# ZJU-FAST-Lab/Implicit-SDF-Planner

Measured on AMD Instinct MI355X. Metric: SDF cost+grad point-evals/sec, higher is better.
Workload: dtype f64; 1 GPU; V3 ESDF-tile sweep: 1 trajectory x 40 pieces x 65 samples/piece, 256^3 fp32 ESDF @ 0.2 m, kernel_size 21, box robot (1.6,0.3,0.3) central-diff grad, occ_thresh = 0, cull off = BASELINE configs[1]; pieces=40, samples_per_piece=65, grid=256, kernel_size=21, collective=none

## Files before the change

implicit-sdf-planner_amd/csrc/dev_math.hpp:

```cpp
#pragma once
#include <hip/hip_runtime.h>

namespace isdf {

template <typename T> struct v3 { T x, y, z; };
using d3 = v3<double>;
using f3 = v3<float>;
struct d4 { double w, x, y, z; };
struct m3 { double a[9]; };

template <typename T> __device__ __forceinline__ v3<T> mkv(T x, T y, T z) { v3<T> r; r.x = x; r.y = y; r.z = z; return r; }
__device__ __forceinline__ d3 mk3(double x, double y, double z) { return mkv<double>(x, y, z); }
template <typename T> __device__ __forceinline__ v3<T> operator+(v3<T> a, v3<T> b) { return mkv<T>(a.x + b.x, a.y + b.y, a.z + b.z); }
template <typename T> __device__ __forceinline__ v3<T> operator-(v3<T> a, v3<T> b) { return mkv<T>(a.x - b.x, a.y - b.y, a.z - b.z); }
template <typename T> __device__ __forceinline__ v3<T> operator*(T s, v3<T> a) { return mkv<T>(s * a.x, s * a.y, s * a.z); }
template <typename T> __device__ __forceinline__ T dot3(v3<T> a, v3<T> b) { return a.x * b.x + a.y * b.y + a.z * b.z; }

#ifdef ISDF_LEAN_MATH
__device__ __forceinline__ double m_sqrt(double x) {
    const double y = __builtin_amdgcn_rsq(fmax(fabs(x), 2.2250738585072014e-308));
    double g = x * y, h = 0.5 * y;
    const double r = fma(-h, g, 0.5);
    g = fma(g, r, g);
    h = fma(h, r, h);
// ... 155 lines not shown
    t.dzt1 = j.y + P.dh_over_m * t.dw1;
    t.dzt2 = j.z + P.dh_over_m * t.dw2;
    t.dz0 = t.ng00 * t.dzt0 + t.ng01 * t.dzt1 + t.ng02 * t.dzt2;
    t.dz1 = t.ng01 * t.dzt0 + t.ng11 * t.dzt1 + t.ng12 * t.dzt2;
    t.dz2 = t.ng02 * t.dzt0 + t.ng12 * t.dzt1 + t.ng22 * t.dzt2;
    t.omg_den = s.z2 + 1.0;
    [[maybe_unused]] const double inv_omg = m_rcp(t.omg_den);
    t.omg_term = ISDF_QUOT(t.dz2, t.omg_den, inv_omg);
}
__device__ __forceinline__ d3 flat_omg(const FlatS &s, const FlatS2 &t) {
    [[maybe_unused]] const double inv_omg = m_rcp(t.omg_den);
    return mk3(-t.dz1 + s.z1 * t.omg_term, t.dz0 - s.z0 * t.omg_term, ISDF_QUOT(s.z1 * t.dz0 - s.z0 * t.dz1, t.omg_den, inv_omg));
}

__device__ __forceinline__ void flat_backward_from(const FlatP &P, d3 v, d3 a, const FlatS &s, const FlatS2 &t, d3 pos_grad, d3 vel_grad,
                                                   d4 quat_grad, d3 omg_grad, d3 &gP, d3 &gV, d3 &gA, d3 &gJ) {
    [[maybe_unused]] const double inv_tilt = m_rcp(s.tilt_den), inv_omg = m_rcp(t.omg_den), inv_ng = m_rcp(t.ng_den), inv_zn = m_rcp(s.zu_norm), inv_cp = m_rcp(s.cp_term);
    const double tilt0b = quat_grad.w, tilt1b = quat_grad.x, tilt2b = quat_grad.y;
    [[maybe_unused]] const double tilt_den_sqr = s.tilt_den * s.tilt_den;
    const double tilt_denb = ISDF_QUOT(s.z1 * tilt1b - s.z0 * tilt2b, tilt_den_sqr, inv_tilt * inv_tilt) + 0.5 * tilt0b;
    const double omg_termb = -s.z0 * omg_grad.y + s.z1 * omg_grad.x;
    double tb = ISDF_QUOT(omg_grad.z, t.omg_den, inv_omg);
    double z1b = t.dz0 * tb;
    const double dz0b = s.z1 * tb + omg_grad.y;
    double z0b = -(t.dz1 * tb);
    const double dz1b = -s.z0 * tb - omg_grad.x;
    const double omg_denb = -ISDF_QUOT((s.z1 * t.dz0 - s.z0 * t.dz1) * tb, t.omg_den, inv_omg) - ISDF_QUOT(ISDF_QUOT(t.dz2 * omg_termb, t.omg_den, inv_omg), t.omg_den, inv_omg);
    tb = -(t.omg_term * omg_grad.y);
    z0b += tb;
    tb = -(t.omg_term * omg_grad.x);
    z0b += ISDF_QUOT(tilt2b, s.tilt_den, inv_tilt);
    z1b += -tb - ISDF_QUOT(tilt1b, s.tilt_den, inv_tilt);
    const double dz2b = ISDF_QUOT(omg_termb, t.omg_den, inv_omg);
    const double z2b = omg_denb + ISDF_QUOT(tilt_denb, s.tilt_den, inv_tilt);

    const double ng02b = t.dzt0 * dz2b + t.dzt2 * dz0b;
    const double dzt0b = t.ng02 * dz2b + t.ng01 * dz1b + t.ng00 * dz0b;
    const double ng12b = t.dzt1 * dz2b + t.dzt2 * dz1b;
    const double dzt1b = t.ng12 * dz2b + t.ng11 * dz1b + t.ng01 * dz0b;
    const double ng22b = t.dzt2 * dz2b;
    const double dzt2b = t.ng22 * dz2b + t.ng12 * dz1b + t.ng02 * dz0b;
    const double ng01b = t.dzt0 * dz1b + t.dzt1 * dz0b;
    const double ng11b = t.dzt1 * dz1b;
    const double ng00b = t.dzt0 * dz0b;
    gJ = mk3(dzt0b, dzt1b, dzt2b);
    const double dw0b = P.dh_over_m * dzt0b, dw1b = P.dh_over_m * dzt1b, dw2b = P.dh_over_m * dzt2b;
    tb = ISDF_QUOT(P.cp * (v.z * dw2b + v.y * dw1b + v.x * dw0b), s.cp_term, inv_cp);
    gA = mk3(s.w_term * dw0b + v.x * tb, s.w_term * dw1b + v.y * tb, s.w_term * dw2b + v.z * tb);
    gV = mk3(t.dw_term * dw0b + a.x * tb, t.dw_term * dw1b + a.y * tb, t.dw_term * dw2b + a.z * tb);
    double cp_termb = -ISDF_QUOT(t.v_dot_a * tb, s.cp_term, inv_cp);
    tb = ISDF_QUOT(ng22b, t.ng_den, inv_ng);
    double zs0b = tb, zs1b = tb;
    double ng_denb = -ISDF_QUOT((s.s0 + s.s1) * tb, t.ng_den, inv_ng);
    const double zu12b = -ISDF_QUOT(ng12b, t.ng_den, inv_ng);
    tb = ISDF_QUOT(ng11b, t.ng_den, inv_ng);
    ng_denb += ISDF_QUOT(ISDF_QUOT(t.zu12 * ng12b, t.ng_den, inv_ng), t.ng_den, inv_ng) - ISDF_QUOT((s.s0 + s.s2) * tb, t.ng_den, inv_ng);
    zs0b += tb;
    double zs2b = tb;
    const double zu02b = -ISDF_QUOT(ng02b, t.ng_den, inv_ng);
    const double zu01b = -ISDF_QUOT(ng01b, t.ng_den, inv_ng);
    tb = ISDF_QUOT(ng00b, t.ng_den, inv_ng);
    ng_denb += ISDF_QUOT(ISDF_QUOT(t.zu02 * ng02b, t.ng_den, inv_ng), t.ng_den, inv_ng) + ISDF_QUOT(ISDF_QUOT(t.zu01 * ng01b, t.ng_den, inv_ng), t.ng_den, inv_ng) - ISDF_QUOT((s.s1 + s.s2) * tb, t.ng_den, inv_ng);
    const double zu_normb = s.zu_sqr_norm * ng_denb - (s.zu2 * z2b + s.zu1 * z1b + s.zu0 * z0b) / s.zu_sqr_norm;
    const double zu_sqr_normb = s.zu_norm * ng_denb + ISDF_QUOT(0.5 * zu_normb, s.zu_norm, inv_zn);
    tb += zu_sqr_normb;
    zs1b += tb;
    zs2b += tb;
    const double zu2b = ISDF_QUOT(z2b, s.zu_norm, inv_zn) + s.zu0 * zu02b + s.zu1 * zu12b + 2 * s.zu2 * zs2b;
    const double w2b = P.dh_over_m * zu2b;
    const double zu1b = ISDF_QUOT(z1b, s.zu_norm, inv_zn) + s.zu2 * zu12b + s.zu0 * zu01b + 2 * s.zu1 * zs1b;
    const double w1b = P.dh_over_m * zu1b;
    zs0b += zu_sqr_normb;
    const double zu0b = ISDF_QUOT(z0b, s.zu_norm, inv_zn) + s.zu2 * zu02b + s.zu1 * zu01b + 2 * s.zu0 * zs0b;
    const double w0b = P.dh_over_m * zu0b;
    const double w_termb = a.z * dw2b + a.y * dw1b + a.x * dw0b + v.z * w2b + v.y * w1b + v.x * w0b;
    gA.x += zu0b; gA.y += zu1b; gA.z += zu2b;
    cp_termb += P.cp * w_termb;
    const double vsb = ISDF_QUOT(0.5 * cp_termb, s.cp_term, inv_cp);
    gV.x += s.w_term * w0b + 2 * v.x * vsb + vel_grad.x;
    gV.y += s.w_term * w1b + 2 * v.y * vsb + vel_grad.y;
    gV.z += s.w_term * w2b + 2 * v.z * vsb + vel_grad.z;
    gP = pos_grad;
}
__device__ __forceinline__ void flat_backward(const FlatP &P, d3 v, d3 a, d3 jer, d3 pos_grad, d3 vel_grad,
                                              d4 quat_grad, d3 omg_grad, d3 &gP, d3 &gV, d3 &gA, d3 &gJ) {
    FlatS s; FlatS2 t;
    flat_core(P, v, a, s);
    flat_core2(P, v, a, jer, s, t);
    flat_backward_from(P, v, a, s, t, pos_grad, vel_grad, quat_grad, omg_grad, gP, gV, gA, gJ);
}

struct Basis { double b0[6], b1[6], b2[6], b3[6], b4[6]; };
__device__ __forceinline__ void poly_basis(double s1, Basis &B) {
    const double s2 = s1 * s1, s3 = s2 * s1, s4 = s2 * s2, s5 = s4 * s1;
    B.b0[0] = 1.0; B.b0[1] = s1; B.b0[2] = s2; B.b0[3] = s3; B.b0[4] = s4; B.b0[5] = s5;
    B.b1[0] = 0.0; B.b1[1] = 1.0; B.b1[2] = 2.0 * s1; B.b1[3] = 3.0 * s2; B.b1[4] = 4.0 * s3; B.b1[5] = 5.0 * s4;
    B.b2[0] = 0.0; B.b2[1] = 0.0; B.b2[2] = 2.0; B.b2[3] = 6.0 * s1; B.b2[4] = 12.0 * s2; B.b2[5] = 20.0 * s3;
    B.b3[0] = 0.0; B.b3[1] = 0.0; B.b3[2] = 0.0; B.b3[3] = 6.0; B.b3[4] = 24.0 * s1; B.b3[5] = 60.0 * s2;
    B.b4[0] = 0.0; B.b4[1] = 0.0; B.b4[2] = 0.0; B.b4[3] = 0.0; B.b4[4] = 24.0; B.b4[5] = 120.0 * s1;
}
template <int K0 = 0> __device__ __forceinline__ d3 ct_beta(const double *__restrict__ c, int ld, const double *b) {
    d3 r;
    double s = 0.0;
#pragma unroll
    for (int k = K0; k < 6; k++) s += c[k] * b[k];
    r.x = s; s = 0.0;
#pragma unroll
    for (int k = K0; k < 6; k++) s += c[ld + k] * b[k];
    r.y = s; s = 0.0;
#pragma unroll
    for (int k = K0; k < 6; k++) s += c[2 * ld + k] * b[k];
    r.z = s;
    return r;
}

struct TrajView { const double *T; const double *C; int N; };
__device__ __forceinline__ int traj_locate(const TrajView &tr, double &t) {
    int idx = 0;
    bool walking = true;
    double last = 0.0;
    for (int k = 0; k < tr.N; k++) {
        const double dur = tr.T[k];
        last = dur;
        walking = walking && (t > dur);
        if (walking) { t -= dur; idx = k + 1; }
        if (!__builtin_amdgcn_ballot_w64(walking)) break;
    }
    if (idx == tr.N) { idx--; t += last; }
    return idx;
}
__device__ __forceinline__ void traj_eval(const TrajView &tr, int piece, double t, d3 &pos, d3 &vel, d3 &acc, d3 &jer) {
    pos = mk3(0, 0, 0); vel = pos; acc = pos; jer = pos;
    double pos_tn = 1.0, vel_tn = 1.0, acc_tn = 1.0, jer_tn = 1.0;
    int vel_n = 1, acc_m = 1, acc_n = 2, jl = 1, jm = 2, jn = 3;
    const int ld = 6 * tr.N;
    const double *c = tr.C + 6 * piece;
#pragma unroll
    for (int power = 0; power <= 5; power++) {
        const d3 ck = mk3(c[power], c[ld + power], c[2 * ld + power]);
        pos = pos + pos_tn * ck;
        pos_tn *= t;
        if (power >= 1) { vel = vel + (vel_n * vel_tn) * ck; vel_tn *= t; vel_n++; }
        if (power >= 2) { acc = acc + (acc_m * acc_n * acc_tn) * ck; acc_tn *= t; acc_m++; acc_n++; }
        if (power >= 3) { jer = jer + (jl * jm * jn * jer_tn) * ck; jer_tn *= t; jl++; jm++; jn++; }
    }
}

__device__ __forceinline__ double wave_sum(double v) {
#pragma unroll
    for (int off = 32; off >= 1; off >>= 1) v += __shfl_xor(v, off, 64);
    return v;
}

__device__ __forceinline__ int wave_sum8_lane(int k) { return ((k & 1) << 3) | (((k >> 1) & 1) << 4) | ((k >> 2) << 5); }
template <int CTRL> __device__ __forceinline__ double dpp_mov_f64(double v) {
    const int lo = __builtin_amdgcn_mov_dpp(__double2loint(v), CTRL, 0xf, 0xf, false);
    const int hi = __builtin_amdgcn_mov_dpp(__double2hiint(v), CTRL, 0xf, 0xf, false);
    return __hiloint2double(hi, lo);
}
__device__ __forceinline__ double swap32_sum(double a, double b) {
    const auto lo = __builtin_amdgcn_permlane32_swap(__double2loint(a), __double2loint(b), false, false);
    const auto hi = __builtin_amdgcn_permlane32_swap(__double2hiint(a), __double2hiint(b), false, false);
    return __hiloint2double(hi[0], lo[0]) + __hiloint2double(hi[1], lo[1]);
}
__device__ __forceinline__ double swap16_sum(double a, double b) {
    const auto lo = __builtin_amdgcn_permlane16_swap(__double2loint(a), __double2loint(b), false, false);
// ... 55 lines not shown
```

implicit-sdf-planner_amd/csrc/isdf_host.hip:

```cpp
#include "isdf_ctx.hpp"
#include "minco_dev.hpp"
#include "lbfgs_host.hpp"
#include <array>
#include <atomic>
#include <map>
#include <dlfcn.h>
#include <chrono>
#include <cmath>
#include <cstdio>
#include <cstring>
#include <functional>
#include <cstdlib>
#include <string>
#include <vector>
#include <new>
#include "fwn_host.hpp"

using namespace isdf;

namespace {
thread_local std::string g_create_error;
}

int isdf_fail(isdf_ctx *c, int code, const char *msg) {
// ... 741 lines not shown
        P.point_partial = c->d_point_partial; P.point_piece = c->d_point_piece; P.point_stat = c->d_point_stat;
        P.point_nr = c->d_point_nr; P.task_buf = c->d_task_buf; P.task_map = c->d_task_map; P.words = c->d_v1_words; P.point_lmask = c->d_point_lmask;
        const bool scan_lpt = !c->env_no_lpt && !fixed_tstar;
        const bool sort_here = c->shape.kind == ISDF_SHAPE_MESH;
        P.scan_ticks = scan_lpt ? c->d_scan_ticks : nullptr; P.scan_order_out = scan_lpt ? c->d_scan_order : nullptr; P.scan_sort_here = (scan_lpt && sort_here) ? 1 : 0;
        const bool order_valid = sort_here || (c->scan_order_b == (long long)b && c->scan_order_e == (long long)e && c->scan_order_epoch == c->points_epoch);
        P.scan_order = (scan_lpt && order_valid) ? c->d_scan_order : nullptr;
        const long long order_b = sort_here ? -1 : b, order_e = sort_here ? -1 : e;
        if (scan_lpt) { c->scan_order_b = c->scan_order_e = -1; }
        P.direct_records = fixed_tstar ? 1 : 0;
        { int rc2 = ensure(c, &c->d_hist, &c->hist_cap, (size_t)N); if (rc2) return rc2; }
        P.hist = c->d_hist;
        P.stats = c->d_stats;
        P.dbg = nullptr;
        if (const char *e = getenv("ISDF_DEBUG_TIMING")) if (e[0] == '1') {
            const size_t need = (size_t)c->M * 7 + (size_t)(N + 1) * 8;
            if (c->dbg_cap < need) {
                if (c->d_dbg) (void)hipFree(c->d_dbg);
                c->d_dbg = nullptr; c->dbg_cap = 0;
                HIPCHK(c, hipMalloc(&c->d_dbg, need * sizeof(unsigned long long)));
                c->dbg_cap = need;
            }
            HIPCHK(c, hipMemsetAsync(c->d_dbg, 0, need * sizeof(unsigned long long), st));
            c->dbg_used = need;
            P.dbg = c->d_dbg;
        }
        if (fixed_tstar) {
            launch_swept_fixed(P, d_tstar, st);
            launch_swept_reduce(P, d_out, st);
            HIPCHK(c, hipGetLastError());
            return ISDF_OK;
        }
        launch_swept_prepare(P, st);
        ProfEvent *ev;
        int rc = prof_begin(c, st, &ev);
        if (rc) return rc;
        launch_swept_sweep(P, st, ev ? ev->a : nullptr, ev ? ev->b : nullptr);
        const bool ev2 = ev && c->prof_secondary;
        if (ev2) { HIPCHK(c, hipEventRecord(ev->c, st)); }
        launch_swept_reduce(P, d_out, st);
        if (ev2) { HIPCHK(c, hipEventRecord(ev->d, st)); }
        HIPCHK(c, hipGetLastError());
        if (scan_lpt) { c->scan_order_b = order_b; c->scan_order_e = order_e; c->scan_order_epoch = c->points_epoch; }
        return ISDF_OK;
    }

    if (cfg.enable_pos && c->shape.kind == ISDF_SHAPE_MESH && c->mesh_depth > isdf::MESH_Q_LEVELS)
        return fail(c, ISDF_ERR_UNSUPPORTED, "mesh hierarchy deeper than 12 levels: the tile sweep (V2 / V3) does not take it (the swept-volume sweep does)");
    if (cfg.enable_pos) {
        if (!c->have_geom) return fail(c, ISDF_ERR_STATE, "grid not set");
        if (cfg.variant == ISDF_V3_ESDF_TILE && !c->d_esdf) return fail(c, ISDF_ERR_STATE, "V3 needs an ESDF grid");
        if (cfg.variant == ISDF_V2_OCC_TILE && !c->d_occ) return fail(c, ISDF_ERR_STATE, "V2 needs an occupancy grid");
    }
    const long long total_pieces = (long long)n_traj * N;
    long long pb, pe;
    shard_range(total_pieces, c->rank, c->world, pb, pe);
    const size_t n_samples = (size_t)total_pieces * (cfg.integral_intervs + 1);
    { int rc0 = isdf_reserve_sweep_buffers(c, total_pieces); if (rc0) return rc0; }
    int rc = ISDF_OK;
    SweepParams P{};
    P.grid = c->grid;
    if (!c->have_geom) { P.grid.X = P.grid.Y = P.grid.Z = 1; P.grid.res = 1.0; }
    P.shape = c->shape;
    fill_flat(cfg, P.flat);
    P.variant = cfg.variant; P.K = cfg.integral_intervs; P.enable_dyn = cfg.enable_dyn; P.enable_pos = cfg.enable_pos;
    P.enable_cull = cfg.enable_cull;
    P.n_traj = n_traj; P.N = N; P.piece_begin = (int)pb; P.piece_end = (int)pe;
    P.bd_half = cfg.kernel_size * P.grid.res / 2;
    P.safety_hor = cfg.safety_hor; P.weight_p = cfg.weight_p; P.weight_v = cfg.weight_v; P.weight_omg = cfg.weight_omg;
    P.weight_theta = cfg.weight_theta;
    P.vel_sqr_max = cfg.vmax * cfg.vmax; P.omg_sqr_max = cfg.omgmax * cfg.omgmax; P.theta_max = cfg.thetamax;
    P.mu = cfg.smoothing_eps; P.inv_mu = 1.0 / cfg.smoothing_eps; P.inv_K = 1.0 / cfg.integral_intervs;
    P.occ_thresh = (float)cfg.occ_thresh;
    P.cull_threshold = 0.0;
    if (cfg.variant == ISDF_V3_ESDF_TILE && cfg.enable_cull && c->shape.bound_radius > 0)
        P.cull_threshold = c->shape.bound_radius + cfg.safety_hor + std::sqrt(3.0) * P.grid.res + (cfg.occ_thresh > 0 ? cfg.occ_thresh : 0.0);
    P.T = d_T; P.coeffs = d_coeffs; P.acc = c->d_acc; P.sample_info = c->d_sample_info; P.piece_cost = c->d_piece_cost;
    P.out = d_out; P.stats = c->d_stats;
    P.dbg = nullptr;
    P.sample_map = (c->d_sample_map && c->sample_map_n == 4 * (((size_t)(pe - pb) * (cfg.integral_intervs + 1) + 3) / 4)) ? c->d_sample_map : nullptr;
    P.dbg_flags = 0;
    if (const char *e = getenv("ISDF_DEBUG_FLAGS")) P.dbg_flags = atoi(e);
    if (const char *e = getenv("ISDF_DEBUG_TIMING")) if (e[0] == '1') {
        const size_t need = n_samples * 8 + (size_t)total_pieces * 4 + 4;
        if (c->dbg_cap < need) {
            if (c->d_dbg) (void)hipFree(c->d_dbg);
            c->d_dbg = nullptr; c->dbg_cap = 0;
            HIPCHK(c, hipMalloc(&c->d_dbg, need * sizeof(unsigned long long)));
            c->dbg_cap = need;
        }
        HIPCHK(c, hipMemsetAsync(c->d_dbg, 0, need * sizeof(unsigned long long), st));
        c->dbg_used = need;
        P.dbg = c->d_dbg;
    }
    if (cfg.enable_pos && c->bits_dirty) {
        const int zw = (c->grid.Z + 31) / 32, xw = (c->grid.X + 31) / 32, yw = (c->grid.Y + 31) / 32;
        const size_t nwz = (size_t)c->grid.X * c->grid.Y * zw, nwx = (size_t)c->grid.Y * c->grid.Z * xw, nwy = (size_t)c->grid.X * c->grid.Z * yw;
        const size_t nw = nwz + nwx + nwy;
        if (c->bits_cap < nw) {
            if (c->d_bits) (void)hipFree(c->d_bits);
            c->d_bits = nullptr; c->bits_cap = 0;
            HIPCHK(c, hipMalloc(&c->d_bits, nw * sizeof(unsigned)));
            c->bits_cap = nw;
        }
        c->grid.ZW = zw; c->grid.XW = xw; c->grid.YW = yw;
        c->grid.bits = c->d_bits; c->grid.bits_x = c->d_bits + nwz; c->grid.bits_y = c->d_bits + nwz + nwx;
        launch_build_bits(c->grid, cfg.variant == ISDF_V3_ESDF_TILE ? 1 : 0, cfg.occ_thresh, c->d_bits, st);
        launch_build_bits_xy(c->grid, cfg.variant == ISDF_V3_ESDF_TILE ? 1 : 0, cfg.occ_thresh, c->d_bits + nwz, c->d_bits + nwz + nwx, st);
        c->bits_dirty = false;
        P.grid = c->grid;
    }
    c->last_P = P; c->have_last_P = true;
    ProfEvent *ev;
    rc = prof_begin(c, st, &ev);
    if (rc) return rc;
    if (ev && !cfg.enable_pos) { ev = nullptr; c->prof_used--; }
    const bool ev2 = ev && c->prof_secondary;
    const bool fused = c->fuse_small && !ev2 && sweep_can_fuse(P);
    {
        int xerr = ISDF_OK;
        if (isdf_xchg_fill(c, &P.xf, (size_t)total_pieces, &xerr)) {
            if (xerr != ISDF_OK) return xerr;
        }
    }
    if (hd) {
        if (!fused || P.xf.world > 1 || P.dbg) return ISDF_DIRECT_NA;
        { int rc1 = ensure_stage(c, (size_t)total_pieces); if (rc1) return rc1; }
        P.out = hd->out; P.host_flag = hd->flags; P.seq = hd->seq;
        if (!hd->via_bar) { P.host_T = hd->T; P.host_coeffs = hd->coeffs; P.stage = c->d_stage; P.stage_flags = c->d_stage_flags; }
        c->last_P = P;
    }
    P.plan_cls_in = nullptr; P.plan_cls_out = nullptr; P.plan_map_out = nullptr; P.plan_zone = 0; P.plan_group = 1;
    P.plan_lr_in = P.plan_hist_in = nullptr; P.plan_lr_out = P.plan_hist_out = nullptr;
    {
        const int K1 = cfg.integral_intervs + 1;
        const long long n_loc = pe - pb, ns_local = n_loc * K1;
        const int nb = (int)((ns_local + 3) / 4);
        P.n_sweep_blocks = nb;
        if (c->n_cus == 0) { hipDeviceProp_t pr; c->n_cus = (hipGetDeviceProperties(&pr, c->device) == hipSuccess && pr.multiProcessorCount > 0) ? pr.multiProcessorCount : 256; }
        const bool no_plan = c->env_no_lpt;
        bool plan = cfg.enable_pos && !no_plan && !P.sample_map && K1 <= 128 && nb > c->n_cus && ns_local < (1LL << 28) && c->shape.kind != ISDF_SHAPE_MESH;
        long long group = n_loc;
        int zone = 0;
        if (plan) {
            if (fused) {
                plan = P.xf.world <= 1 && pb == 0 && pe == total_pieces && ns_local <= PLAN_GROUP_MAX_SAMPLES;
                zone = c->n_cus;
            } else if (nb <= sweep_resident_blocks(P, c->n_cus) && ns_local <= PLAN_GROUP_MAX_SAMPLES) {
                zone = c->n_cus;
            } else if (ns_local > PLAN_GROUP_MAX_SAMPLES) {
                group = N;
                plan = (long long)N * K1 <= PLAN_GROUP_MAX_SAMPLES && pb % N == 0 && pe % N == 0;
            }
        }
        if (!plan) c->plan_k = 0;
        else {
            const size_t ns_cap = (size_t)4 * nb, np_cap = (size_t)n_loc;
            if (c->plan_ns_cap < ns_cap || c->plan_np_cap < np_cap) {
                HIPCHK(c, hipStreamSynchronize(st));
                for (void *q : {(void *)c->d_plan_cls, (void *)c->d_plan_map, (void *)c->d_plan_lr, (void *)c->d_plan_hist}) if (q) (void)hipFree(q);
                c->d_plan_cls = nullptr; c->d_plan_map = nullptr; c->d_plan_lr = nullptr; c->d_plan_hist = nullptr;
                c->plan_ns_cap = c->plan_np_cap = 0; c->plan_k = 0; c->plan_cur = 0;
                const size_t nsc = std::max(ns_cap, (size_t)4096), npc = std::max(np_cap, (size_t)256);
                HIPCHK(c, hipMalloc(&c->d_plan_cls, 2 * nsc));
                HIPCHK(c, hipMalloc(&c->d_plan_map, 2 * nsc * sizeof(int)));
                HIPCHK(c, hipMalloc(&c->d_plan_lr, 2 * nsc * sizeof(unsigned short)));
                HIPCHK(c, hipMalloc(&c->d_plan_hist, 2 * npc * PLAN_CLASSES * sizeof(unsigned short)));
// ... 1187 lines not shown
```

implicit-sdf-planner_amd/csrc/tile_sweep.hip:

```cpp
#define ISDF_LEAN_MATH 1
#ifndef ISDF_SWEEP_STATS
#define ISDF_SWEEP_STATS 0
#endif
#include "isdf_internal.hpp"
#include "dev_mesh.hpp"

namespace isdf {

constexpr int SW_LIST_CAP = 1024;
constexpr int MQ_BLOCK = 16;
constexpr int SW_PASS = 8;
constexpr int SW_NEAR_CAP = 512;
constexpr float TS_FILTER_EPS = 2e-3f;

__device__ __forceinline__ void wave_lds_sync() {
    __builtin_amdgcn_fence(__ATOMIC_RELEASE, "wavefront");
    __builtin_amdgcn_wave_barrier();
    __builtin_amdgcn_fence(__ATOMIC_ACQUIRE, "wavefront");
}

__device__ __forceinline__ bool in_map(const DevGrid &G, double x, double y, double z) {
    if (x < G.bmin[0] || y < G.bmin[1] || z < G.bmin[2]) return false;
    if (x > G.bmax[0] || y > G.bmax[1] || z > G.bmax[2]) return false;
    return true;
// ... 1072 lines not shown
        if (qv < n) {
            const unsigned ent = P.mq_entries[(size_t)it * MQ_BLOCK + qv];
            const int gx = q->lo[0] + (int)(ent & 1023u), gy = q->lo[1] + (int)((ent >> 10) & 1023u), gz = q->lo[2] + (int)(ent >> 20);
            const d3 ctr = mk3((gx + 0.5) * G.res + G.bmin[0], (gy + 0.5) * G.res + G.bmin[1], (gz + 0.5) * G.res + G.bmin[2]);
            const d3 pos = mk3(q->pos[0], q->pos[1], q->pos[2]);
            pm = ctr - pos;
            prel = mat_tmul(R, pm);
            want = !(fmax(fmax(fabs(prel.x), fabs(prel.y)), fabs(prel.z)) > P.bd_half);
        }
        double sdf = 0.0;
        d3 g = mk3(0, 0, 0);
        const bool below = mesh_sdf_grad_below_quad(P.shape.mesh, MeshFrames{&s_mframes[wave][0], MESH_Q_LEVELS}, prel, want, P.safety_hor, sdf, g);
        const bool owner = (lane & 3) == 0;
        bool is_grad = false;
        if (owner && want && below) {
            double f = 0.0, df = 0.0;
            smoothed_l1_inv(P.safety_hor - sdf, P.mu, P.inv_mu, f, df);
            if (f > 0.0) {
                is_grad = true;
                v[0] = f;
                d4 quat; quat.w = q->quat[0]; quat.x = q->quat[1]; quat.y = q->quat[2]; quat.z = q->quat[3];
                const d3 wg = mat_mul(R, g);
                v[1] = df * wg.x; v[2] = df * wg.y; v[3] = df * wg.z;
                const d4 sq = quat_step_grad(quat, g, pm);
                v[4] = -df * sq.w; v[5] = -df * sq.x; v[6] = -df * sq.y; v[7] = -df * sq.z;
            }
        }
        wave_sum8(v, lane);
        const int comp = ((lane >> 3) & 1) | (((lane >> 4) & 1) << 1) | ((lane >> 5) << 2);
        const int np = __popcll(__ballot(owner && want)), ng = __popcll(__ballot(is_grad));
        double *o = P.mq_res + (size_t)it * 10;
        if ((lane & 7) == 0) o[comp] = v[0];
        if (lane == 1) { o[8] = (double)np; o[9] = (double)ng; }
    }
}
__global__ __launch_bounds__(256) void mesh_sum_kernel(const SweepParams P) {
    const long long n_samples = (long long)(P.piece_end - P.piece_begin) * (P.K + 1);
    const long long sl = (long long)blockIdx.x * blockDim.x + threadIdx.x;
    if (sl >= n_samples) return;
    const int w = P.mq_sample_n[sl], nb = w & 0x3fffffff;
    double tot[ACC_STRIDE] = {0, 0, 0, 0, 0, 0, 0, 0};
    int np = 0, ng = 0;
    for (int bk = 0; bk < nb; bk++) {
        const double *o = P.mq_res + (size_t)P.mq_sample_items[(size_t)sl * P.mq_kmax + bk] * 10;
#pragma unroll
        for (int k = 0; k < ACC_STRIDE; k++) tot[k] += o[k];
        np += (int)o[8]; ng += (int)o[9];
    }
#pragma unroll
    for (int k = 0; k < ACC_STRIDE; k++) P.acc[(size_t)sl * ACC_STRIDE + k] = tot[k];
    P.sample_info[2 * sl] = np;
    P.sample_info[2 * sl + 1] = ng | ((w & (1 << 30)) ? (int)0x80000000 : 0);
}

__global__ __launch_bounds__(256) void stats_kernel(const SweepParams P) {
    const int K1 = P.K + 1;
    const long long n_samples = (long long)(P.piece_end - P.piece_begin) * K1;
    unsigned long long culled = 0, pairs = 0, grads = 0;
    if (P.enable_pos)
        for (long long s = (long long)blockIdx.x * blockDim.x + threadIdx.x; s < n_samples; s += (long long)gridDim.x * blockDim.x) {
            const int a = P.sample_info[2 * s], b = P.sample_info[2 * s + 1];
            pairs += (unsigned)a; grads += (unsigned)(b & 0x7fffffff);
            if (b < 0) culled++;
        }
    if (culled) atomicAdd(&P.stats[1], culled);
    if (pairs) atomicAdd(&P.stats[2], pairs);
    if (grads) atomicAdd(&P.stats[3], grads);
    if (blockIdx.x == 0 && threadIdx.x == 0) atomicAdd(&P.stats[0], (unsigned long long)n_samples);
}

template <bool EARLY, bool XF> __device__ __forceinline__ void tail_piece(const SweepParams &P, const int t, double (*s_val)[PARTIAL_STRIDE + 1]) {
    const int K1 = P.K + 1;
    const int tid = threadIdx.x;
    const int n_own = P.piece_end - P.piece_begin;
    int gp = t;
    if constexpr (XF) gp = t < n_own ? P.piece_begin + t : (t - n_own < P.piece_begin ? t - n_own : t);
    const int b = gp / P.N, i = gp - b * P.N;
    const size_t ostride = (size_t)1 + 19 * (size_t)P.N;
    const int p0 = max(P.piece_begin, b * P.N) - b * P.N, p1 = min(P.piece_end, (b + 1) * P.N) - b * P.N;
    double *const o = P.out + (size_t)b * ostride;
    double *const my_board = XF ? P.xf.board[P.xf.rank] + (size_t)P.xf.parity * P.xf.parity_stride : nullptr;
    bool lost = false;
    const bool mine = i >= p0 && i < p1;
    unsigned long long *const dbg = (ISDF_SWEEP_STATS && P.dbg && mine) ? P.dbg + (size_t)(P.piece_end - P.piece_begin) * K1 * 8 + (size_t)(gp - P.piece_begin) * 4 : nullptr;
    if (!mine) {
        const int q = tid;
        if constexpr (XF) {
            if (q < 19) {
                double v;
                unsigned long long deadline = 0ull;
                lost = !xslot_take(my_board + (size_t)gp * XF_ROW + q, v, P.xf.timeout_ticks, deadline);
                if (q == 18) o[1 + i] = v;
                else { const int d = q / 6, r = q - 6 * d; o[1 + P.N + (size_t)d * 6 * P.N + 6 * i + r] = v; }
            }
        } else {
            if (q == 18) o[1 + i] = 0.0;
            else if (q < 18) { const int d = q / 6, r = q - 6 * d; o[1 + P.N + (size_t)d * 6 * P.N + 6 * i + r] = 0.0; }
            else if (q == 19 && p1 <= p0 && i == 0) o[0] = 0.0;
            return;
        }
    } else {
    if constexpr (!EARLY) {
        if (P.host_T) {
            __shared__ int s_staged;
            if (tid == 0) s_staged = stage_wait(P, gp) ? 1 : 0;
            __syncthreads();
            lost = lost || !s_staged;
        }
    }
    const PieceIn pin = piece_in(P, b, i);
    const double *c = pin.c;
    const int ld = pin.ld;
    const double integral_frac = P.inv_K;
    const double step = pin.T * integral_frac;
    double colsum = 0.0;
    unsigned long long tl_c0 = 0, tl_marks = 0;
    if (dbg && tid == 0) { dbg[0] = wall_clock64(); tl_c0 = clock64(); }
#define TL_MARK(k) do { if (dbg && tid == 0) tl_marks |= (((clock64() - tl_c0) >> 4) & 0xFFFFull) << (16 * (k)); } while (0)
    for (int j0 = 0; j0 < (EARLY ? K1 : min(K1, 1)); j0 += TL_THREADS) {
        const int j = j0 + tid;
        if (tid < TL_THREADS && j < K1) {
            const long long s = (long long)gp * K1 + j;
            double *const ap = P.acc + (size_t)(s - (long long)P.piece_begin * K1) * ACC_STRIDE;
            double ab[EARLY ? ACC_STRIDE : 1];
            if (EARLY && P.enable_pos) {
#pragma unroll
                for (int q = 0; q < ACC_STRIDE; q++) ab[q] = ap[q];
            }
            d3 vel, acc3, jer0;
            {
                Basis B;
                poly_basis(j * step, B);
                vel = ct_beta<1>(c, ld, B.b1); acc3 = ct_beta<2>(c, ld, B.b2); jer0 = ct_beta<3>(c, ld, B.b3);
            }
            TL_MARK(0);
            double pena = 0.0;
            d3 gradVel = mk3(0, 0, 0), gradPos = gradVel, gradOmg = gradVel;
            d4 gradQuat; gradQuat.w = gradQuat.x = gradQuat.y = gradQuat.z = 0.0;
            FlatS fs; FlatS2 ft;
            flat_core(P.flat, vel, acc3, fs);
            flat_core2(P.flat, vel, acc3, jer0, fs, ft);
            if (P.enable_dyn) {
                const d4 quat = flat_quat(fs);
                const d3 omg = flat_omg(fs, ft);
                const double cos_theta = 1.0 - 2.0 * (quat.x * quat.x + quat.y * quat.y);
                const double violaVel = dot3(vel, vel) - P.vel_sqr_max;
                const double violaOmg = dot3(omg, omg) - P.omg_sqr_max;
                const double violaTheta = acos(cos_theta) - P.theta_max;
                double pe, pd;
                if (smoothed_l1_inv(violaVel, P.mu, P.inv_mu, pe, pd)) {
                    gradVel = (P.weight_v * pd * 2.0) * vel;
                    pena += P.weight_v * pe;
                }
                if (smoothed_l1_inv(violaOmg, P.mu, P.inv_mu, pe, pd)) {
                    gradOmg = (P.weight_omg * pd * 2.0) * omg;
                    pena += P.weight_omg * pe;
                }
                if (smoothed_l1_inv(violaTheta, P.mu, P.inv_mu, pe, pd)) {
                    const double f = P.weight_theta * pd / sqrt(1.0 - cos_theta * cos_theta) * 4.0;
                    gradQuat.x += f * quat.x;
                    gradQuat.y += f * quat.y;
                    pena += P.weight_theta * pe;
                }
            }
            TL_MARK(1);
            if (P.enable_pos) {
                double a[ACC_STRIDE];
                if constexpr (EARLY) {
#pragma unroll
                    for (int q = 0; q < ACC_STRIDE; q++) { a[q] = ab[q]; ap[q] = __longlong_as_double((long long)SLOT_EMPTY); }
                } else {
                    unsigned long long v[ACC_STRIDE];
                    bool ok = false;
                    for (int spin = 0; spin < SLOT_SPIN_MAX; spin++) {
                        ok = true;
#pragma unroll
                        for (int q = 0; q < ACC_STRIDE; q++) { v[q] = slot_peek(ap + q); ok = ok && v[q] != SLOT_EMPTY; }
                        if (ok) break;
                        __builtin_amdgcn_s_sleep(2);
                    }
                    lost = lost || !ok;
#pragma unroll
                    for (int q = 0; q < ACC_STRIDE; q++) { a[q] = __longlong_as_double((long long)v[q]); slot_clear(ap + q); }
                }
                if (a[0] > 0.0) {
                    gradPos.x += P.weight_p * a[1]; gradPos.y += P.weight_p * a[2]; gradPos.z += P.weight_p * a[3];
                    gradQuat.w += P.weight_p * a[4]; gradQuat.x += P.weight_p * a[5];
                    gradQuat.y += P.weight_p * a[6]; gradQuat.z += P.weight_p * a[7];
                    pena += P.weight_p * a[0];
                }
            }
            d3 gP, gV, gA, gJ;
            TL_MARK(2);
            flat_backward_from(P.flat, vel, acc3, fs, ft, gradPos, gradVel, gradQuat, gradOmg, gP, gV, gA, gJ);
            TL_MARK(3);
            const double node = (j == 0 || j == P.K) ? 0.5 : 1.0;
            const double alpha = j * integral_frac;
            double *o = s_val[tid];
            double s1 = j * step;
            asm volatile("" : "+v"(s1));
            Basis B;
            poly_basis(s1, B);
            const d3 jer = ct_beta<3>(c, ld, B.b3), sna = ct_beta<4>(c, ld, B.b4);
            const double gPv[3] = {gP.x, gP.y, gP.z}, gVv[3] = {gV.x, gV.y, gV.z}, gAv[3] = {gA.x, gA.y, gA.z}, gJv[3] = {gJ.x, gJ.y, gJ.z};
#pragma unroll
            for (int d = 0; d < 3; d++)
#pragma unroll
                for (int r = 0; r < 6; r++) {
                    double v = B.b0[r] * gPv[d];
                    if (r >= 1) v += B.b1[r] * gVv[d];
                    if (r >= 2) v += B.b2[r] * gAv[d];
                    if (r >= 3) v += B.b3[r] * gJv[d];
                    o[d * 6 + r] = v * node * step;
                }
            o[18] = (dot3(gP, vel) + dot3(gV, acc3) + dot3(gA, jer) + dot3(gJ, sna)) * alpha * node * step + node * integral_frac * pena;
            o[19] = node * step * pena;
        }
        __syncthreads();
        {
            const int n = min(TL_THREADS, K1 - j0);
            const int col = tid % PARTIAL_STRIDE, grp = tid / PARTIAL_STRIDE;
            double part = 0.0;
            if (grp < TL_GROUPS) for (int row = grp; row < n; row += TL_GROUPS) part += s_val[row][col];
            __syncthreads();
            if (grp < TL_GROUPS) s_val[grp][col] = part;
            __syncthreads();
            if (tid < PARTIAL_STRIDE) {
#pragma unroll
                for (int g = 0; g < TL_GROUPS; g++) colsum += s_val[g][tid];
            }
        }
        __syncthreads();
    }
    if (dbg && tid == 0) { dbg[2] = tl_marks; dbg[3] = (clock64() - tl_c0) >> 4; }
#undef TL_MARK
    if (P.host_flag) lost = __syncthreads_or(lost ? 1 : 0) != 0;
    if (tid < PARTIAL_STRIDE) {
        const int q = tid;
        if (q < 19) {
            if (q == 18) o[1 + i] = colsum;
            else { const int d = q / 6, r = q - 6 * d; o[1 + P.N + (size_t)d * 6 * P.N + 6 * i + r] = colsum; }
            if constexpr (XF) {
                for (int r = 0; r < P.xf.world; r++)
                    if (r != P.xf.rank) xslot_publish(P.xf.board[r] + (size_t)P.xf.parity * P.xf.parity_stride + (size_t)gp * XF_ROW + q, colsum);
            }
        } else {
            if (P.host_flag) { if (lost && P.stats) atomicMax(&P.stats[4], 1ull); __builtin_amdgcn_fence(__ATOMIC_RELEASE, ""); }
            if constexpr (XF) {
                for (int r = 0; r < P.xf.world; r++) xslot_publish(P.xf.board[r] + (size_t)P.xf.parity * P.xf.parity_stride + (size_t)gp * XF_ROW + 19, colsum);
            } else slot_publish(&P.piece_cost[gp], colsum);
        }
    }
    }
    if (lost && P.stats) atomicMax(&P.stats[4], 1ull);
    bool collector;
    int k0, k1;
    if constexpr (XF) {
        const int first = b * P.N, last = first + P.N - 1;
        const int t_last = (last >= P.piece_begin && last < P.piece_end) ? last - P.piece_begin : (last < P.piece_begin ? last + n_own : last);
        const int below = P.piece_begin - 1;
        const int t_below = (below >= first && below <= last) ? below + n_own : -1;
        collector = t == max(t_last, t_below);
        k0 = 0; k1 = P.N;
    } else {
        collector = i == p1 - 1;
        k0 = p0; k1 = p1;
    }
    if (collector && tid < 64) {
        double sum = 0.0;
        bool gone = false;
        unsigned long long deadline = 0ull;
        for (int k = k0 + tid; k < k1; k += 64) {
            double v;
            if constexpr (XF) gone = !xslot_take(my_board + ((size_t)b * P.N + k) * XF_ROW + 19, v, P.xf.timeout_ticks, deadline) || gone;
            else {
                double *slot = &P.piece_cost[(size_t)b * P.N + k];
                unsigned long long bits = slot_peek(slot);
                for (int spin = 0; bits == SLOT_EMPTY && spin < SLOT_SPIN_MAX; spin++) {
                    __builtin_amdgcn_s_sleep(1);
                    bits = slot_peek(slot);
                }
                gone = gone || bits == SLOT_EMPTY;
                slot_clear(slot);
                v = __longlong_as_double((long long)bits);
            }
            sum += v;
        }
        sum = wave_sum(sum);
        if (__ballot(gone) != 0ull) { sum = __longlong_as_double(0x7FF8000000000000ll); if (tid == 0 && P.stats) atomicMax(&P.stats[4], 1ull); }
        if (tid == 0) o[0] = sum;
    }
    if constexpr (!XF) {
        if (P.host_flag && collector && tid == 0) {
            __builtin_amdgcn_fence(__ATOMIC_ACQUIRE, "agent");
            const unsigned long long ovf = P.stats ? __hip_atomic_load(&P.stats[4], __ATOMIC_RELAXED, __HIP_MEMORY_SCOPE_AGENT) : 0ull;
            __hip_atomic_store(&P.host_flag[b], P.seq | (ovf ? HOST_FLAG_OVERFLOW : 0ull), __ATOMIC_RELEASE, __HIP_MEMORY_SCOPE_SYSTEM);
        }
    }
    if (dbg && tid == 0) dbg[1] = wall_clock64();
}

constexpr int TL_LAUNCH_THREADS = TL_THREADS + 64;
template <bool XF> __device__ __forceinline__ void tail_plan(const SweepParams &P) {
    if (!(P.plan_cls_in || P.plan_lr_in) || (P.dbg_flags & 2) || (int)(threadIdx.x >> 6) != TL_THREADS / 64) return;
    int gp = (int)blockIdx.x;
    if constexpr (XF) { const int n_own = P.piece_end - P.piece_begin, t = gp; gp = t < n_own ? P.piece_begin + t : (t - n_own < P.piece_begin ? t - n_own : t); }
    if (gp >= P.piece_begin && gp < P.piece_end) plan_wave(P, gp - P.piece_begin, (int)(threadIdx.x & 63));
}
__global__ __launch_bounds__(TL_LAUNCH_THREADS) void tail_kernel(const SweepParams P) {
    __shared__ double s_val[TL_THREADS][PARTIAL_STRIDE + 1];
    tail_plan<false>(P);
    tail_piece<true, false>(P, (int)blockIdx.x, s_val);
}
__global__ __launch_bounds__(TL_LAUNCH_THREADS) void tail_kernel_xf(const SweepParams P) {
    __shared__ double s_val[TL_THREADS][PARTIAL_STRIDE + 1];
    tail_plan<true>(P);
    tail_piece<true, true>(P, (int)blockIdx.x, s_val);
}

static int fused_max_blocks() {
    static const int v = [] { const char *e = getenv("ISDF_FUSE_MAX_BLOCKS"); const int n = e ? atoi(e) : 0; return n > 0 ? n : 3 * 256; }();
    return v;
}

int sweep_resident_blocks(const SweepParams &P, int n_cus) {
    const bool ident = P.shape.d.ident != 0;
    const int kind = P.shape.kind == ISDF_SHAPE_MESH ? ISDF_SHAPE_MESH : P.shape.kind;
    return sweep_waves_per_simd(kind, kind == ISDF_SHAPE_MESH ? false : ident) * n_cus;
}

bool sweep_can_fuse(const SweepParams &P) {
    if (!P.enable_pos || P.shape.kind == ISDF_SHAPE_MESH || P.shape.d.ident == 0) return false;
    const long long n_samples = (long long)(P.piece_end - P.piece_begin) * (P.K + 1);
    if (n_samples <= 0 || P.K + 1 > TL_THREADS) return false;
    return (n_samples + SW_SAMPLES - 1) / SW_SAMPLES + (long long)(P.piece_end - P.piece_begin) <= fused_max_blocks() && (long long)P.n_traj * P.N <= 8 * fused_max_blocks();
}

static int sweep_target_blocks_mesh() {
    static int cus = 0;
    if (cus == 0) {
        int dev = 0, n = 0;
        cus = 256;
        if (hipGetDevice(&dev) == hipSuccess && hipDeviceGetAttribute(&n, hipDeviceAttributeMultiprocessorCount, dev) == hipSuccess && n > 0) cus = n;
    }
    return 5 * cus;
}
void launch_sweep(const SweepParams &P0, hipStream_t stream, hipEvent_t ev_start, hipEvent_t ev_stop, bool fused) {
    SweepParams P = P0;
    const long long n_samples = (long long)(P.piece_end - P.piece_begin) * (P.K + 1);
    if (n_samples <= 0 || !P.enable_pos) return;
    P.n_sweep_blocks = (int)((n_samples + SW_SAMPLES - 1) / SW_SAMPLES);
    const dim3 grid((unsigned)(P.n_sweep_blocks + (fused ? P.n_traj * P.N : 0))), block(64 * SW_SAMPLES);
    const bool ident = P.shape.d.ident != 0;
    if (!fused) hipLaunchKernelGGL(pose_kernel, dim3((unsigned)((n_samples + POSE_THREADS - 1) / POSE_THREADS)), dim3(POSE_THREADS), 0, stream, P);
#define ISDF_LAUNCH_SWEEP(K, I, F) hipExtLaunchKernelGGL((sweep_kernel<K, I, F>), grid, block, 0, stream, ev_start, ev_stop, 0, P)
#define ISDF_SWEEP_CASE(K) case K: if (fused) ISDF_LAUNCH_SWEEP(K, true, true); else if (ident) ISDF_LAUNCH_SWEEP(K, true, false); else ISDF_LAUNCH_SWEEP(K, false, false); break;
    switch (P.shape.kind) {
    ISDF_SWEEP_CASE(ISDF_SHAPE_TORUS) ISDF_SWEEP_CASE(ISDF_SHAPE_CAPPEDTORUS) ISDF_SWEEP_CASE(ISDF_SHAPE_CAPPEDCONE)
    ISDF_SWEEP_CASE(ISDF_SHAPE_ROUNDEDCONE) ISDF_SWEEP_CASE(ISDF_SHAPE_WIREFRAMEBOX) ISDF_SWEEP_CASE(ISDF_SHAPE_BENDLINEAR)
    ISDF_SWEEP_CASE(ISDF_SHAPE_TWISTBOX) ISDF_SWEEP_CASE(ISDF_SHAPE_BENDBOX) ISDF_SWEEP_CASE(ISDF_SHAPE_TABLE)
    ISDF_SWEEP_CASE(ISDF_SHAPE_TREFOIL) ISDF_SWEEP_CASE(ISDF_SHAPE_SMOOTHDIFFERENCE) ISDF_SWEEP_CASE(ISDF_SHAPE_SMOOTHINTERSECTION)
    ISDF_SWEEP_CASE(ISDF_SHAPE_CSG) ISDF_SWEEP_CASE(ISDF_SHAPE_BOX)
    case ISDF_SHAPE_MESH:
        if (P.mq_items) {
            hipExtLaunchKernelGGL((sweep_kernel<ISDF_SHAPE_MESH, false, false>), grid, block, 0, stream, ev_start, nullptr, 0, P);
            hipLaunchKernelGGL(mesh_exact_kernel, dim3((unsigned)std::min<long long>((long long)sweep_target_blocks_mesh(), ((long long)P.mq_cap + SW_SAMPLES - 1) / SW_SAMPLES)), block, 0, stream, P);
            hipExtLaunchKernelGGL(mesh_sum_kernel, dim3((unsigned)((n_samples + 255) / 256)), dim3(256), 0, stream, nullptr, ev_stop, 0, P);
        } else ISDF_LAUNCH_SWEEP(ISDF_SHAPE_MESH, false, false);
        break;
    default: if (fused) ISDF_LAUNCH_SWEEP(-1, true, true); else if (ident) ISDF_LAUNCH_SWEEP(-1, true, false); else ISDF_LAUNCH_SWEEP(-1, false, false); break;
    }
// ... 66 lines not shown
```

Before: 163.1 million point-evals/s.

## Precompute flatness backward and tilt sensitivities before waiting on ESDF accumulators

```diff
diff --git a/implicit-sdf-planner_amd/csrc/dev_math.hpp b/implicit-sdf-planner_amd/csrc/dev_math.hpp
--- a/implicit-sdf-planner_amd/csrc/dev_math.hpp
+++ b/implicit-sdf-planner_amd/csrc/dev_math.hpp
@@ -261,6 +261,27 @@
     gV.z += s.w_term * w2b + 2 * v.z * vsb + vel_grad.z;
     gP = pos_grad;
 }
+struct TiltSens { double A[3][3], V[3][3]; };
+__device__ __forceinline__ void flat_tilt_sens(const FlatP &P, d3 v, const FlatS &s, const FlatS2 &t, TiltSens &S) {
+    [[maybe_unused]] const double inv_t = m_rcp(s.tilt_den), inv_cp = m_rcp(s.cp_term);
+    const double it = ISDF_QUOT(1.0, s.tilt_den, inv_t);
+    const double it3 = it * it * it;
+    const double ng[3][3] = {{t.ng00, t.ng01, t.ng02}, {t.ng01, t.ng11, t.ng12}, {t.ng02, t.ng12, t.ng22}};
+#pragma unroll
+    for (int r = 0; r < 3; r++) {
+        S.A[r][0] = 0.5 * it * ng[r][2];
+        S.A[r][1] = s.z1 * it3 * ng[r][2] - it * ng[r][1];
+        S.A[r][2] = it * ng[r][0] - s.z0 * it3 * ng[r][2];
+    }
+    const double k = ISDF_QUOT(P.cp, s.cp_term, inv_cp);
+#pragma unroll
+    for (int c = 0; c < 3; c++) {
+        const double u = k * (v.x * S.A[0][c] + v.y * S.A[1][c] + v.z * S.A[2][c]);
+        S.V[0][c] = P.dh_over_m * (s.w_term * S.A[0][c] + v.x * u);
+        S.V[1][c] = P.dh_over_m * (s.w_term * S.A[1][c] + v.y * u);
+        S.V[2][c] = P.dh_over_m * (s.w_term * S.A[2][c] + v.z * u);
+    }
+}
 __device__ __forceinline__ void flat_backward(const FlatP &P, d3 v, d3 a, d3 jer, d3 pos_grad, d3 vel_grad,
                                               d4 quat_grad, d3 omg_grad, d3 &gP, d3 &gV, d3 &gA, d3 &gJ) {
     FlatS s; FlatS2 t;
diff --git a/implicit-sdf-planner_amd/csrc/isdf_host.hip b/implicit-sdf-planner_amd/csrc/isdf_host.hip
--- a/implicit-sdf-planner_amd/csrc/isdf_host.hip
+++ b/implicit-sdf-planner_amd/csrc/isdf_host.hip
@@ -847,7 +847,7 @@
     P.dbg_flags = 0;
     if (const char *e = getenv("ISDF_DEBUG_FLAGS")) P.dbg_flags = atoi(e);
     if (const char *e = getenv("ISDF_DEBUG_TIMING")) if (e[0] == '1') {
-        const size_t need = n_samples * 8 + (size_t)total_pieces * 4 + 4;
+        const size_t need = n_samples * 8 + (size_t)total_pieces * 8 + 4;
         if (c->dbg_cap < need) {
             if (c->d_dbg) (void)hipFree(c->d_dbg);
             c->d_dbg = nullptr; c->dbg_cap = 0;
diff --git a/implicit-sdf-planner_amd/csrc/tile_sweep.hip b/implicit-sdf-planner_amd/csrc/tile_sweep.hip
--- a/implicit-sdf-planner_amd/csrc/tile_sweep.hip
+++ b/implicit-sdf-planner_amd/csrc/tile_sweep.hip
@@ -1178,7 +1178,7 @@
     double *const my_board = XF ? P.xf.board[P.xf.rank] + (size_t)P.xf.parity * P.xf.parity_stride : nullptr;
     bool lost = false;
     const bool mine = i >= p0 && i < p1;
-    unsigned long long *const dbg = (ISDF_SWEEP_STATS && P.dbg && mine) ? P.dbg + (size_t)(P.piece_end - P.piece_begin) * K1 * 8 + (size_t)(gp - P.piece_begin) * 4 : nullptr;
+    unsigned long long *const dbg = (ISDF_SWEEP_STATS && P.dbg && mine) ? P.dbg + (size_t)(P.piece_end - P.piece_begin) * K1 * 8 + (size_t)(gp - P.piece_begin) * 8 : nullptr;
     if (!mine) {
         const int q = tid;
         if constexpr (XF) {
@@ -1223,41 +1223,64 @@
 #pragma unroll
                 for (int q = 0; q < ACC_STRIDE; q++) ab[q] = ap[q];
             }
-            d3 vel, acc3, jer0;
+            d3 vel, acc3, jer0, sna0;
             {
                 Basis B;
                 poly_basis(j * step, B);
-                vel = ct_beta<1>(c, ld, B.b1); acc3 = ct_beta<2>(c, ld, B.b2); jer0 = ct_beta<3>(c, ld, B.b3);
+                vel = ct_beta<1>(c, ld, B.b1); acc3 = ct_beta<2>(c, ld, B.b2); jer0 = ct_beta<3>(c, ld, B.b3); sna0 = ct_beta<4>(c, ld, B.b4);
             }
             TL_MARK(0);
             double pena = 0.0;
-            d3 gradVel = mk3(0, 0, 0), gradPos = gradVel, gradOmg = gradVel;
-            d4 gradQuat; gradQuat.w = gradQuat.x = gradQuat.y = gradQuat.z = 0.0;
-            FlatS fs; FlatS2 ft;
-            flat_core(P.flat, vel, acc3, fs);
-            flat_core2(P.flat, vel, acc3, jer0, fs, ft);
-            if (P.enable_dyn) {
-                const d4 quat = flat_quat(fs);
-                const d3 omg = flat_omg(fs, ft);
-                const double cos_theta = 1.0 - 2.0 * (quat.x * quat.x + quat.y * quat.y);
-                const double violaVel = dot3(vel, vel) - P.vel_sqr_max;
-                const double violaOmg = dot3(omg, omg) - P.omg_sqr_max;
-                const double violaTheta = acos(cos_theta) - P.theta_max;
-                double pe, pd;
-                if (smoothed_l1_inv(violaVel, P.mu, P.inv_mu, pe, pd)) {
-                    gradVel = (P.weight_v * pd * 2.0) * vel;
-                    pena += P.weight_v * pe;
-                }
-                if (smoothed_l1_inv(violaOmg, P.mu, P.inv_mu, pe, pd)) {
-                    gradOmg = (P.weight_omg * pd * 2.0) * omg;
-                    pena += P.weight_omg * pe;
-                }
-                if (smoothed_l1_inv(violaTheta, P.mu, P.inv_mu, pe, pd)) {
-                    const double f = P.weight_theta * pd / sqrt(1.0 - cos_theta * cos_theta) * 4.0;
-                    gradQuat.x += f * quat.x;
-                    gradQuat.y += f * quat.y;
-                    pena += P.weight_theta * pe;
-                }
+            d3 gP = mk3(0, 0, 0), gV, gA, gJ;
+            TiltSens S;
+            bool tilt = true;
+            if constexpr (EARLY) tilt = P.enable_pos && ab[0] > 0.0;
+            {
+                d3 gradVel = mk3(0, 0, 0), gradOmg = gradVel;
+                d4 gradQuat; gradQuat.w = gradQuat.x = gradQuat.y = gradQuat.z = 0.0;
+                FlatS fs; FlatS2 ft;
+                flat_core(P.flat, vel, acc3, fs);
+                flat_core2(P.flat, vel, acc3, jer0, fs, ft);
+                if (P.enable_dyn) {
+                    const d4 quat = flat_quat(fs);
+                    const d3 omg = flat_omg(fs, ft);
+                    const double cos_theta = 1.0 - 2.0 * (quat.x * quat.x + quat.y * quat.y);
+                    const double violaVel = dot3(vel, vel) - P.vel_sqr_max;
+                    const double violaOmg = dot3(omg, omg) - P.omg_sqr_max;
+                    const double violaTheta = acos(cos_theta) - P.theta_max;
+                    double pe, pd;
+                    if (smoothed_l1_inv(violaVel, P.mu, P.inv_mu, pe, pd)) {
+                        gradVel = (P.weight_v * pd * 2.0) * vel;
+                        pena += P.weight_v * pe;
+                    }
+                    if (smoothed_l1_inv(violaOmg, P.mu, P.inv_mu, pe, pd)) {
+                        gradOmg = (P.weight_omg * pd * 2.0) * omg;
+                        pena += P.weight_omg * pe;
+                    }
+                    if (smoothed_l1_inv(violaTheta, P.mu, P.inv_mu, pe, pd)) {
+                        const double f = P.weight_theta * pd / sqrt(1.0 - cos_theta * cos_theta) * 4.0;
+                        gradQuat.x += f * quat.x;
+                        gradQuat.y += f * quat.y;
+                        pena += P.weight_theta * pe;
+                    }
+                }
+                flat_backward_from(P.flat, vel, acc3, fs, ft, gP, gradVel, gradQuat, gradOmg, gP, gV, gA, gJ);
+                if (tilt) flat_tilt_sens(P.flat, vel, fs, ft, S);
+            }
+            double e18 = dot3(gV, acc3) + dot3(gA, jer0) + dot3(gJ, sna0), r18[3] = {0.0, 0.0, 0.0};
+            if (tilt) {
+#pragma unroll
+                for (int q = 0; q < 3; q++)
+                    r18[q] = S.V[0][q] * acc3.x + S.V[1][q] * acc3.y + S.V[2][q] * acc3.z + S.A[0][q] * jer0.x + S.A[1][q] * jer0.y + S.A[2][q] * jer0.z;
+            }
+            {
+                double *const w[] = {&gV.x, &gV.y, &gV.z, &gA.x, &gA.y, &gA.z, &gJ.x, &gJ.y, &gJ.z, &e18, &r18[0], &r18[1], &r18[2], &pena};
+#pragma unroll
+                for (double *x : w) asm volatile("" : "+v"(*x));
+#pragma unroll
+                for (int r = 0; r < 3; r++)
+#pragma unroll
+                    for (int q = 0; q < 3; q++) asm volatile("" : "+v"(S.A[r][q]), "+v"(S.V[r][q]));
             }
             TL_MARK(1);
             if (P.enable_pos) {
@@ -1279,17 +1302,21 @@
 #pragma unroll
                     for (int q = 0; q < ACC_STRIDE; q++) { a[q] = __longlong_as_double((long long)v[q]); slot_clear(ap + q); }
                 }
+                if (dbg) atomicMax(&dbg[4], wall_clock64());
                 if (a[0] > 0.0) {
-                    gradPos.x += P.weight_p * a[1]; gradPos.y += P.weight_p * a[2]; gradPos.z += P.weight_p * a[3];
-                    gradQuat.w += P.weight_p * a[4]; gradQuat.x += P.weight_p * a[5];
-                    gradQuat.y += P.weight_p * a[6]; gradQuat.z += P.weight_p * a[7];
+                    gP = mk3(P.weight_p * a[1], P.weight_p * a[2], P.weight_p * a[3]);
+                    const double qw = P.weight_p * a[4], qx = P.weight_p * a[5], qy = P.weight_p * a[6];
+                    gA.x += S.A[0][0] * qw + S.A[0][1] * qx + S.A[0][2] * qy;
+                    gA.y += S.A[1][0] * qw + S.A[1][1] * qx + S.A[1][2] * qy;
+                    gA.z += S.A[2][0] * qw + S.A[2][1] * qx + S.A[2][2] * qy;
+                    gV.x += S.V[0][0] * qw + S.V[0][1] * qx + S.V[0][2] * qy;
+                    gV.y += S.V[1][0] * qw + S.V[1][1] * qx + S.V[1][2] * qy;
+                    gV.z += S.V[2][0] * qw + S.V[2][1] * qx + S.V[2][2] * qy;
+                    e18 += dot3(gP, vel) + (r18[0] * qw + r18[1] * qx + r18[2] * qy);
                     pena += P.weight_p * a[0];
                 }
             }
-            d3 gP, gV, gA, gJ;
             TL_MARK(2);
-            flat_backward_from(P.flat, vel, acc3, fs, ft, gradPos, gradVel, gradQuat, gradOmg, gP, gV, gA, gJ);
-            TL_MARK(3);
             const double node = (j == 0 || j == P.K) ? 0.5 : 1.0;
             const double alpha = j * integral_frac;
             double *o = s_val[tid];
@@ -1297,7 +1324,6 @@
             asm volatile("" : "+v"(s1));
             Basis B;
             poly_basis(s1, B);
-            const d3 jer = ct_beta<3>(c, ld, B.b3), sna = ct_beta<4>(c, ld, B.b4);
             const double gPv[3] = {gP.x, gP.y, gP.z}, gVv[3] = {gV.x, gV.y, gV.z}, gAv[3] = {gA.x, gA.y, gA.z}, gJv[3] = {gJ.x, gJ.y, gJ.z};
 #pragma unroll
             for (int d = 0; d < 3; d++)
@@ -1309,7 +1335,7 @@
                     if (r >= 3) v += B.b3[r] * gJv[d];
                     o[d * 6 + r] = v * node * step;
                 }
-            o[18] = (dot3(gP, vel) + dot3(gV, acc3) + dot3(gA, jer) + dot3(gJ, sna)) * alpha * node * step + node * integral_frac * pena;
+            o[18] = e18 * alpha * node * step + node * integral_frac * pena;
             o[19] = node * step * pena;
         }
         __syncthreads();
@@ -1317,7 +1343,15 @@
             const int n = min(TL_THREADS, K1 - j0);
             const int col = tid % PARTIAL_STRIDE, grp = tid / PARTIAL_STRIDE;
             double part = 0.0;
-            if (grp < TL_GROUPS) for (int row = grp; row < n; row += TL_GROUPS) part += s_val[row][col];
+            if (grp < TL_GROUPS) {
+                for (int row0 = grp; row0 < n; row0 += 4 * TL_GROUPS) {
+                    double v[4];
+#pragma unroll
+                    for (int k = 0; k < 4; k++) v[k] = s_val[min(row0 + k * TL_GROUPS, TL_THREADS - 1)][col];
+#pragma unroll
+                    for (int k = 0; k < 4; k++) if (row0 + k * TL_GROUPS < n) part += v[k];
+                }
+            }
             __syncthreads();
             if (grp < TL_GROUPS) s_val[grp][col] = part;
             __syncthreads();
@@ -1336,6 +1370,7 @@
         if (q < 19) {
             if (q == 18) o[1 + i] = colsum;
             else { const int d = q / 6, r = q - 6 * d; o[1 + P.N + (size_t)d * 6 * P.N + 6 * i + r] = colsum; }
+            if (dbg && q == 0) dbg[5] = wall_clock64();
             if constexpr (XF) {
                 for (int r = 0; r < P.xf.world; r++)
                     if (r != P.xf.rank) xslot_publish(P.xf.board[r] + (size_t)P.xf.parity * P.xf.parity_stride + (size_t)gp * XF_ROW + q, colsum);
@@ -1345,6 +1380,7 @@
             if constexpr (XF) {
                 for (int r = 0; r < P.xf.world; r++) xslot_publish(P.xf.board[r] + (size_t)P.xf.parity * P.xf.parity_stride + (size_t)gp * XF_ROW + 19, colsum);
             } else slot_publish(&P.piece_cost[gp], colsum);
+            if (dbg) dbg[6] = wall_clock64();
         }
     }
     }
@@ -1383,6 +1419,7 @@
             sum += v;
         }
         sum = wave_sum(sum);
+        if (dbg && tid == 0) dbg[7] = wall_clock64();
         if (__ballot(gone) != 0ull) { sum = __longlong_as_double(0x7FF8000000000000ll); if (tid == 0 && P.stats) atomicMax(&P.stats[4], 1ull); }
         if (tid == 0) o[0] = sum;
     }
```

Result: faster. 169.8 million point-evals/s, median of 6 (+4.1%).
